# invictus717/MetaTransformer

Hardware: AMD Instinct MI355X
Metric: encoder samples/sec at B=256,N=197,C=768 (Base) (higher is better)
Workload: dtype bf16; 1 GPU; BASELINE config 2: Meta-Transformer-Base forward+backward+AdamW, tokens [256,197,768] bf16 per GPU, 12L/768d/12h, fp32 master weights, random init N(0,0.02); mode=train, per_gpu_batch=256, global_batch=256, parallelism=single

## Files before the change

### metatransformer_amd/csrc/api.hip

```cpp
#include "common.h"
#include <stdarg.h>
#include <mutex>
#include <vector>

static thread_local char g_err[512] = "";

void me_set_error(const char* fmt, ...) {
    va_list ap;
    va_start(ap, fmt);
    vsnprintf(g_err, sizeof(g_err), fmt, ap);
    va_end(ap);
}

extern "C" int me_abi_version(void) { return ME_ABI_VERSION; }
extern "C" const char* me_last_error(void) { return g_err; }
extern "C" const char* me_build_arch(void) { return "gfx950"; }

extern "C" int me_device_info(int dev, int* num_cus, int* lds_bytes, int* clock_mhz, char* name, int name_len) {
    hipDeviceProp_t prop;
    hipError_t e = hipGetDeviceProperties(&prop, dev);
    if (e != hipSuccess) {
        me_set_error("me_device_info: %s", hipGetErrorString(e));
        return ME_ERR_HIP;
    }
    if (num_cus) *num_cus = prop.multiProcessorCount;
    if (lds_bytes) *lds_bytes = (int)prop.maxSharedMemoryPerMultiProcessor;
    if (clock_mhz) *clock_mhz = prop.clockRate / 1000;
    if (name && name_len > 0) {
        snprintf(name, (size_t)name_len, "%s (%s)", prop.name, prop.gcnArchName);
    }
    return ME_OK;
}

namespace {
struct ProfEntry { int op, dt; int64_t M, N, K; hipEvent_t e0, e1; int plan; };
std::mutex g_prof_mu;
std::vector<ProfEntry> g_prof;
bool g_prof_on = false;
}

ProfScope::ProfScope(int op_, int dt_, int64_t M_, int64_t N_, int64_t K_, hipStream_t s) : stream(s), op(op_), dt(dt_), M(M_), N(N_), K(K_) {
    if (!g_prof_on) return;
    if (hipEventCreate(&e0) != hipSuccess) { e0 = nullptr; return; }
    (void)hipEventRecord(e0, stream);
}
ProfScope::~ProfScope() {
    if (!e0) return;
    hipEvent_t e1 = nullptr;
    if (hipEventCreate(&e1) != hipSuccess) { (void)hipEventDestroy(e0); return; }
    (void)hipEventRecord(e1, stream);
    std::lock_guard<std::mutex> lk(g_prof_mu);
    g_prof.push_back(ProfEntry{op, dt, M, N, K, e0, e1, plan});
}

extern "C" int me_gemm_profile_enable(int on) {
    std::lock_guard<std::mutex> lk(g_prof_mu);
    for (auto& e : g_prof) { (void)hipEventDestroy(e.e0); (void)hipEventDestroy(e.e1); }
    g_prof.clear();
    g_prof_on = on != 0;
    return ME_OK;
}

extern "C" int me_gemm_profile_read(me_gemm_profile_rec* out, int max) {
    std::lock_guard<std::mutex> lk(g_prof_mu);
    int n = 0;
    for (auto& e : g_prof) {
        float ms = 0.f;
        (void)hipEventSynchronize(e.e1);
        (void)hipEventElapsedTime(&ms, e.e0, e.e1);
        if (out && n < max) out[n] = me_gemm_profile_rec{e.op, e.dt, e.M, e.N, e.K, ms, e.plan};
        ++n;
        (void)hipEventDestroy(e.e0);
        (void)hipEventDestroy(e.e1);
    }
    g_prof.clear();
    return n;
}
```

### metatransformer_amd/csrc/block.hip

```cpp
#include "gemm_host.h"
#include "attention_host.h"
#include <string.h>
#include <stdlib.h>
#include <atomic>
#include <map>
#include <mutex>

namespace {

struct SideCtx {
    hipStream_t side = nullptr;
    hipEvent_t fork[4] = {nullptr, nullptr, nullptr, nullptr}, join = nullptr;
    bool failed = false;
};
std::atomic<int> g_wgrad_overlap{1};
bool wgrad_overlap_on() { return g_wgrad_overlap.load() != 0; }
constexpr size_t kMaxSideCtx = 64;
SideCtx* side_ctx(hipStream_t main) {
    static std::mutex mu;
    static std::map<std::pair<int, hipStream_t>, SideCtx> ctxs;
    hipStreamCaptureStatus st = hipStreamCaptureStatusNone;
    if (hipStreamIsCapturing(main, &st) != hipSuccess || st != hipStreamCaptureStatusNone) return nullptr;
    int dev = 0;
    if (hipStreamGetDevice(main, &dev) != hipSuccess) (void)hipGetDevice(&dev);
// ... 2 lines not shown
    SideCtx& c = ctxs[std::make_pair(dev, main)];
    if (c.failed) return nullptr;
    if (!c.side) {
        int cur = dev;
        (void)hipGetDevice(&cur);
        if (cur != dev && hipSetDevice(dev) != hipSuccess) { c.failed = true; return nullptr; }
        bool ok = hipStreamCreateWithFlags(&c.side, hipStreamNonBlocking) == hipSuccess;
        for (int i = 0; ok && i < 4; ++i) ok = hipEventCreateWithFlags(&c.fork[i], hipEventDisableTiming) == hipSuccess;
        ok = ok && hipEventCreateWithFlags(&c.join, hipEventDisableTiming) == hipSuccess;
        if (cur != dev) (void)hipSetDevice(cur);
        if (!ok) { c.failed = true; c.side = nullptr; return nullptr; }
    }
    return &c;
}

inline size_t align256(size_t v) { return (v + 255) & ~(size_t)255; }

struct Dims {
    int64_t M;
    int C, C3, Hd, hd;
    size_t esz, rsz;
};
int get_dims(const me_block_desc* d, Dims& s, const char* fn) {
    ME_CHECK_ARG(d != nullptr, "%s: null descriptor", fn);
    ME_CHECK_ARG((me_dtype_ok(d->dtype) || d->dtype == ME_BF16X3) && me_dtype_ok(d->res_dtype), "%s: bad dtype", fn);
    ME_CHECK_ARG(d->B > 0 && d->N > 0 && d->C > 0 && d->heads > 0 && d->hidden > 0 && d->C % d->heads == 0,
                 "%s: bad shape B=%d N=%d C=%d heads=%d hidden=%d", fn, d->B, d->N, d->C, d->heads, d->hidden);
    s.M = (int64_t)d->B * d->N;
    s.C = d->C; s.C3 = 3 * d->C; s.Hd = d->hidden; s.hd = d->C / d->heads;
    s.esz = d->dtype == ME_BF16X3 ? 6 : me_dtype_size(d->dtype); s.rsz = me_dtype_size(d->res_dtype);
// ... 43 lines not shown
        if (cs) g.colsum_a = reinterpret_cast<float*>(dummy_mem);
        const size_t b = me_gemm_workspace_bytes(&g);
        if (b > w) w = b;
    };
    probe(ME_GEMM_NT, s.M, s.C3, s.C, d->dtype, false);
    probe(ME_GEMM_NT, s.M, s.C, s.C, d->res_dtype, false);
    probe(ME_GEMM_NT, s.M, s.Hd, s.C, d->dtype, false);
    probe(ME_GEMM_NT, s.M, s.C, s.Hd, d->res_dtype, false);
    if (backward) {
        probe(ME_GEMM_NT, s.M, s.C, s.C3, d->dtype, false);
        probe(ME_GEMM_NT, s.M, s.C, s.Hd, d->dtype, false);
        probe(ME_GEMM_TN, s.C3, s.C, s.M, ME_F32, true);
        probe(ME_GEMM_TN, s.C, s.C, s.M, ME_F32, true);
        probe(ME_GEMM_TN, s.Hd, s.C, s.M, ME_F32, true);
        probe(ME_GEMM_TN, s.C, s.Hd, s.M, ME_F32, true);
    }
    return align256(w);
}

size_t aux_scratch(const Dims& s) {
    size_t a = me_layernorm_bwd_workspace(s.C), b = me_colsum_workspace(s.Hd > s.C3 ? s.Hd : s.C3);
    return align256(a > b ? a : b);
}

bool wants_fold(const me_block_desc* d) {
    return d->dtype != ME_BF16X3 && d->qkv_wf && d->fc1_wf && d->qkv_s && d->qkv_c && d->fc1_s && d->fc1_c && d->res_dtype == d->dtype;
}
size_t stats_scratch(const Dims& s) { return 2 * align256(me_row_stats_partial_bytes(s.M, s.C)) + 2 * align256((size_t)s.M * 8); }
bool emits_stats(const me_block_desc* d, const Dims& s) {
    if (!wants_fold(d) || d->gamma1 || d->gamma2 || s.C % ME_STATS_GROUP) return false;
// ... 406 lines not shown
        if (!dW && !dB) return ME_OK;
        int r = fork(fk);
        if (r) return r;
        if (dW) {
            gemm_desc(g, ME_GEMM_TN, dt, n_out, n_in, s.M, dOut, n_out, In, n_in, dW, n_in, gr->w_dtype);
            g.beta = beta; g.workspace = wgws; g.workspace_bytes = (int64_t)gsz;
            const bool fuse = dB && me_gemm_fuses_colsum(&g);
            if (fuse) g.colsum_a = dB;
            r = me_gemm(&g, wstream);
            if (r) return r;
            if (fuse) return ME_OK;
        }
        if (dB) return me_colsum(dOut, dt, n_out, s.M, n_out, dB, gr->accumulate, waws, wstream);
        return ME_OK;
    };

    const void* dyc = dy;
    if (rdt != dt) {
        if ((rc = me_cast(dy, rdt, dy_c, dt, s.M * s.C, stream))) return rc;
        dyc = dy_c;
    }
    if ((rc = wgrad(0, dyc, s.C, v.a, s.Hd, gr->fc2_w, gr->fc2_b))) return join(rc);
    if ((rc = nt(dyc, s.C, d->fc2_wt, dh, s.Hd, v.hpre))) return join(rc);
    if ((rc = wgrad(1, dh, s.Hd, v.xn2, s.C, gr->fc1_w, gr->fc1_b))) return join(rc);
    if ((rc = nt(dh, s.Hd, d->fc1_wt, dxn, s.C, nullptr))) return join(rc);
    rc = me_ln_bwd_deferred(dxn, dt, v.x1, rdt, v.mean2, v.rstd2, d->ln2_g, dy, rdt, dx1, rdt, gr->ln2_g, gr->ln2_b, gr->accumulate, s.M,
                            s.C, ln2_ws, stream, &folds[0]);
    if (rc) return join(rc);
    const void* dx1c = dx1;
    if (rdt != dt) {
        if ((rc = me_cast(dx1, rdt, dx1_c, dt, s.M * s.C, stream))) return join(rc);
        dx1c = dx1_c;
    }
    if ((rc = wgrad(2, dx1c, s.C, v.o, s.C, gr->proj_w, gr->proj_b))) return join(rc);
    if ((rc = nt(dx1c, s.C, d->proj_wt, dout, s.C, nullptr))) return join(rc);
    rc = me_attention_bwd(v.qkv, s.C3, v.o, s.C, dout, s.C, v.lse, delta, dqkv, s.C3, d->B, d->N, d->heads, s.hd, d->scale, dt, 0.f, 0, stream);
    if (rc) return join(rc);
    if ((rc = wgrad(3, dqkv, s.C3, v.xn1, s.C, gr->qkv_w, gr->qkv_b))) return join(rc);
    if ((rc = nt(dqkv, s.C3, d->qkv_wt, dxn, s.C, nullptr))) return join(rc);
    rc = me_ln_bwd_deferred(dxn, dt, x, rdt, v.mean1, v.rstd1, d->ln1_g, dx1, rdt, dx, rdt, gr->ln1_g, gr->ln1_b, gr->accumulate, s.M, s.C,
                            aws, stream, &folds[1]);
    if (rc) return join(rc);
    return join(me_ln_bwd_fold_sets(folds, 2, s.C, stream));
}

extern "C" int me_block_bwd_overlap(int enable) {
    const int prev = wgrad_overlap_on() ? 1 : 0;
    g_wgrad_overlap.store(enable ? 1 : 0);
    return prev;
}

extern "C" int me_encoder_fwd(const me_block_desc* blocks, int n_blocks, const void* x, void* y, void* pingpong, void* workspace,
                              size_t workspace_bytes, void* stream) {
// ... 37 lines not shown
```

### metatransformer_amd/csrc/common.h

```cpp
#pragma once
constexpr int ME_POL_LN_ST = 0;
constexpr int ME_POL_LN_LD = 0;
constexpr int ME_POL_ATTN_ST = 0;
constexpr int ME_POL_SLAB = 0;
#define ME_NT_LOAD(POL, ptr) ((POL) ? __builtin_nontemporal_load(ptr) : *(ptr))
#define ME_NT_STORE(POL, val, ptr) do { if (POL) __builtin_nontemporal_store((val), (ptr)); else *(ptr) = (val); } while (0)
#include <hip/hip_runtime.h>
#include <stdint.h>
#include <stdio.h>
#include "../../include/metaenc.h"

typedef __bf16 bf16_t;
typedef __attribute__((ext_vector_type(8))) __bf16 bf16x8;
typedef __attribute__((ext_vector_type(4))) __bf16 bf16x4;
typedef __attribute__((ext_vector_type(2))) __bf16 bf16x2;
typedef __attribute__((ext_vector_type(16))) float f32x16;
typedef __attribute__((ext_vector_type(4))) float f32x4;
typedef __attribute__((ext_vector_type(2))) float f32x2;
typedef __attribute__((ext_vector_type(4))) uint32_t u32x4;
constexpr float ME_GG8_LO = -0.13f, ME_GG8_STEP = 1.26f / 255.0f;
constexpr int ME_STATS_GROUP = 256;
typedef __attribute__((ext_vector_type(2))) uint32_t u32x2;

#define ME_WAVE 64
// ... 30 lines not shown
    static int n = 0;
    if (!n) {
        int dev = 0;
        (void)hipGetDevice(&dev);
        if (hipDeviceGetAttribute(&n, hipDeviceAttributeMultiprocessorCount, dev) != hipSuccess || n <= 0) n = 256;
    }
    return n;
}

struct ProfScope {
    hipEvent_t e0 = nullptr;
    hipStream_t stream;
    int op, dt;
    int64_t M, N, K;
    int plan = 0;
    ProfScope(int op, int dt, int64_t M, int64_t N, int64_t K, hipStream_t stream);
    ~ProfScope();
};

static inline size_t me_dtype_size(int dt) { return dt == ME_F32 ? 4 : dt == ME_GG8 ? 1 : 2; }
static inline bool me_dtype_ok(int dt) { return dt == ME_F32 || dt == ME_BF16; }
static inline bool me_storage_dtype_ok(int dt) { return me_dtype_ok(dt) || dt == ME_F16; }
static inline bool me_out_dtype_ok(int dt) { return me_dtype_ok(dt) || dt == ME_BF16X3; }
static inline bool me_is_planes(int dt) { return dt == ME_BF16X3 || dt == ME_BF16X2; }

constexpr int LN_FOLD_SETS = 4;
struct me_ln_fold_set { const float* partial; int nrows; float* dgamma; float* dbeta; int accumulate; };
struct me_ln_fold_batch { me_ln_fold_set set[LN_FOLD_SETS]; int cols; };
int me_ln_bwd_deferred(const void* dy, int dy_dtype, const void* x, int x_dtype, const float* mean, const float* rstd, const float* gamma,
                       const void* dres, int dres_dtype, void* dx, int dx_dtype, float* dgamma, float* dbeta, int accumulate_affine,
// ... 179 lines not shown
```

### metatransformer_amd/csrc/gemm.hip

```cpp
#include "gemm_common.h"
#include <string.h>
#include <algorithm>
#include <atomic>

namespace {

constexpr int BM = 128;
constexpr int BN = 128;
constexpr int ROWB = 128;
constexpr int TILE_BYTES = BM * ROWB;
constexpr int NT = 256;

__device__ __forceinline__ int lds_off(int row, int byteoff) {
    const int chunk = byteoff >> 4;
    return row * ROWB + (((chunk ^ ((row >> 1) & 7)) << 4) | (byteoff & 15));
}

struct Stage { u32x4 v[4]; };

template <typename T>
__device__ __forceinline__ void load_nt(Stage& s, const T* __restrict__ S, int64_t ld, int64_t nrows, int64_t K,
                                        int64_t r0, int64_t k0, int tid) {
    constexpr int E = 16 / sizeof(T);
#pragma unroll
// ... 333 lines not shown
                if (!gelu && res == 2) ME_FOLD(true, 2, 1, false, false);
            }
        }
        if (p.beta == 0.0f && !colsum_out && !bias && !gelu && res == 0) {
            if (p.c_dtype == ME_BF16) ME_FOLD(false, 0, 0, false, false);
            else ME_FOLD(false, 0, 1, false, false);
        }
    }
#undef ME_FOLD
    if (p.act == ME_ACT_NONE && !p.preact && !p.aux && !p.row_affine)
        hipLaunchKernelGGL(splitk_reduce_kernel<true>, grid, dim3(256), 0, stream, p, slabs, S, cs_part, n_part, colsum_out, sstride);
    else
        hipLaunchKernelGGL(splitk_reduce_kernel<false>, grid, dim3(256), 0, stream, p, slabs, S, cs_part, n_part, colsum_out, sstride);
}

struct GemmPlan {
    GemmFamily family = GEMM_G128;
    int bn = 0;
    int bm = 128;
    int kstep = 0;
    int split_k = 1;
    int ksteps_per_split = 0;
    size_t ws_bytes = 0;
    int64_t tail_rows = 0;
    int tail_split = 1, tail_ksteps = 0;
    int sk_wgs = 0, sk_upt = 0, sk_levels = 0, sk_l1 = 0;
};

std::atomic<int> g_reserved_cus{0};

// ... 33 lines not shown
        const int64_t tiles = ((d->M + 255) / 256) * ((d->N + 255) / 256);
        const int nkt = (int)((d->K + 63) / 64);
        const int reserved = g_reserved_cus.load();
        const int slots = 256 - (reserved > 0 ? (reserved < 128 ? reserved : 128) : 0);
        int s = (int)(slots / tiles);
        if (s < 1) s = 1;
        int ktp = (nkt + s - 1) / s;
        ktp += ktp & 1;
        if (ktp < 2) ktp = 2;
        pl.ksteps_per_split = ktp;
        pl.split_k = (nkt + ktp - 1) / ktp;
        int slabs = pl.split_k;
        const int upt = (nkt + 1) / 2;
        const int S = (int)(slots / tiles), E = (int)(slots - S * tiles);
        if (reserved > 0 && S >= 1 && E > 0 && tiles * upt >= 2 * (int64_t)slots && tiles * upt < (1ll << 30)) {
            int L1 = (int)(tiles * upt / slots);
            {
                auto tail = [&](int l1) { return S * l1 > upt ? (int64_t)1 << 40 : std::max<int64_t>(l1, (tiles * (int64_t)(upt - S * l1) + E - 1) / E); };
                if (tail(L1 + 1) < tail(L1)) L1 += 1;
            }
            const int Ul = upt - S * L1;
            int smax = S;
            for (int t = 0; t < (int)tiles; ++t) smax = std::max(smax, S + sk_left_parts(t, E, Ul, tiles * (int64_t)Ul));
            if (allow_sk && L1 >= 1) { pl.sk_wgs = slots; pl.sk_upt = upt; pl.sk_levels = S; pl.sk_l1 = L1; pl.split_k = smax; }
            slabs = std::max(slabs, smax);
        }
        pl.ws_bytes = (size_t)slabs * (size_t)g3_tn_slab_stride(d->M, d->N) * sizeof(float);
        if (d->colsum_a)
            pl.ws_bytes += (size_t)slabs * (size_t)((d->N + 255) / 256) * (size_t)d->M * sizeof(float);
    } else if (d->op == ME_GEMM_TN) {
        pl.bn = (d->N % 256 == 0 || d->N > 512) ? 256 : 128;
        const int64_t tiles = pl.bn == 256 ? t256 : t128;
        int s = (int)(SLOTS / tiles);
        if (s < 1) s = 1;
        const int min_steps = 512 / pl.kstep;
// ... 284 lines not shown
}

int gemm_fill_params(const me_gemm_desc* d, GemmParams& p) { return fill_params(d, p); }

extern "C" int me_gemm(const me_gemm_desc* d, void* stream_) {
    hipStream_t stream = reinterpret_cast<hipStream_t>(stream_);
    ProfScope prof(d ? d->op : 0, d ? d->ab_dtype : 0, d ? d->M : 0, d ? d->N : 0, d ? d->K : 0, stream);
    return gemm_impl(d, stream, &prof.plan);
}

int gemm_tn_with_launcher(const me_gemm_desc* d, hipStream_t stream, GemmTnLaunch launch, const void* ctx) {
    ProfScope prof(d ? d->op : 0, d ? d->ab_dtype : 0, d ? d->M : 0, d ? d->N : 0, d ? d->K : 0, stream);
    return gemm_impl(d, stream, &prof.plan, launch, ctx);
}

extern "C" int me_gemm_reserve_cus(int cus) {
    const int c = cus < 0 ? 0 : (cus > 128 ? 128 : cus);
    return g_reserved_cus.exchange(c);
}

extern "C" size_t me_gemm_workspace_bytes(const me_gemm_desc* d) {
    GemmRoute r;
    return route_gemm(d, r) == ME_OK ? r.pl.ws_bytes : 0;
}

int gemm_tn_is_g3(const me_gemm_desc* d) {
    GemmRoute r;
    return d && d->op == ME_GEMM_TN && route_gemm(d, r) == ME_OK && r.pl.family == GEMM_G3;
}

// ... 28 lines not shown
```

### metatransformer_amd/csrc/gemm3.hip

```cpp
#include "gemm3_core.h"

namespace {
constexpr int G3_ROWOP_AHEAD = 4;
constexpr int G3_ROWOP_AHEAD_HALF = 4;
constexpr int G3_ROWOP_AHEAD_STATS = 4;

template <int EPI, bool WRAP = false>
__global__ __launch_bounds__(512) __attribute__((amdgpu_waves_per_eu(2, 2))) void gemm_g3_kernel(const GemmParams p) {
    extern __shared__ __attribute__((aligned(16))) char smem[];
    const int tid = threadIdx.x, lane = tid & 63;
    const int wave = __builtin_amdgcn_readfirstlane(tid >> 6);
    const int wr = wave >> 2;

    const int nwg = gridDim.x, bid = blockIdx.x;
    const int xcd = bid & 7, slot = bid >> 3;
    const int F = p.g3_full_tiles;
    const int nf = (F >> 3) + (xcd < (F & 7) ? 1 : 0);
    const int base_f = xcd * (F >> 3) + (xcd < (F & 7) ? xcd : (F & 7));
    int tile, part = -1;
    if (slot < nf) {
        tile = base_f + slot;
    } else {
        const int base_all = xcd * (nwg >> 3) + (xcd < (nwg & 7) ? xcd : (nwg & 7));
        const int tid_ = base_all - base_f + (slot - nf);
// ... 698 lines not shown
            c0 += __shfl_xor(c0, 16, 64); c0 += __shfl_xor(c0, 32, 64);
            c1 += __shfl_xor(c1, 16, 64); c1 += __shfl_xor(c1, 32, 64);
            if (lane < 16) {
                float* row = p.colsum_ws + (int64_t)cs_row * p.M;
                const int wcol = wave & 3;
                const int64_t ma = m0 + wr * 128 + wcol * 16 + lane, mb = ma + 64;
                if (ma < p.M) row[ma] = c0;
                if (mb < p.M) row[mb] = c1;
            }
        }
        g3_epilogue<5>(p, s, m0, n0, g3_lane_now(), reinterpret_cast<float*>(p.C) + (int64_t)part * p.slab_stride, 0);
        u0 = ue;
    }
}


unsigned* g3r_tickets(hipStream_t stream) {
    constexpr int SETS = 64, SET_WORDS = 8 * 16;
    struct Pool {
        unsigned* base = nullptr;
        bool failed = false;
        int next = 0;
        std::map<hipStream_t, int> idx;
    };
    static std::mutex mu;
    static std::map<int, Pool> pools;
    hipStreamCaptureStatus st = hipStreamCaptureStatusNone;
    if (hipStreamIsCapturing(stream, &st) != hipSuccess || st != hipStreamCaptureStatusNone) return nullptr;
    int dev = 0;
    if (hipStreamGetDevice(stream, &dev) != hipSuccess) (void)hipGetDevice(&dev);
// ... 76 lines not shown
    const int nwg = p.tiles_m * p.tiles_n * p.split_k;
    hipLaunchKernelGGL(gemm_g3tn_kernel, dim3((unsigned)nwg), dim3(512), G3_LDS, stream, p);
    ME_CHECK_LAUNCH("me_gemm(g3 tn)");
    return ME_OK;
}

int launch_g3_tn_sk(const GemmParams& p, hipStream_t stream) {
    static OncePerDevice once;
    if (once.need())
        (void)hipFuncSetAttribute(reinterpret_cast<const void*>(&gemm_g3tn_sk_kernel), hipFuncAttributeMaxDynamicSharedMemorySize, G3_LDS);
    hipLaunchKernelGGL(gemm_g3tn_sk_kernel, dim3((unsigned)p.sk_wgs), dim3(512), G3_LDS, stream, p);
    ME_CHECK_LAUNCH("me_gemm(g3 tn, balanced partition)");
    return ME_OK;
}

bool g3_tn_supported(const GemmParams& p) {
    return p.M % 8 == 0 && p.N % 8 == 0 && p.lda % 8 == 0 && p.ldb % 8 == 0 && p.K * p.lda * 2 < (1ll << 31) &&
           p.K * p.ldb * 2 < (1ll << 31);
}

bool g3_supported(const GemmParams& p, int op) {
    if (op != ME_GEMM_NT) return false;
    if (p.K % (2 * G3_BK) != 0 || p.N % 8 != 0) return false;
    if (256 * p.lda * 2 >= (1ll << 31) || 256 * p.ldb * 2 >= (1ll << 31)) return false;
    return true;
}

int g3_cu_count() { return device_cus(); }

G3Form g3_form(const GemmParams& p, int cus) {
// ... 61 lines not shown
```

### metatransformer_amd/csrc/gemm_common.h

```cpp
#pragma once
#include "common.h"
#include "gemm_host.h"

struct GemmParams {
    const void* A; const void* B; void* C;
    int64_t M, N, K, lda, ldb, ldc;
    int c_dtype, act;
    int flags;
    float alpha, beta;
    const float* bias; const float* colscale;
    void* preact; int64_t ldpre; int preact_dtype;
    const void* aux; int64_t ldaux; int aux_dtype;
    const void* residual; int64_t ldres; int res_dtype;
    int64_t res_row_mod, out_group_rows, out_group_stride, out_row_offset;
    int tiles_m, tiles_n;
    int split_k, ksteps_per_split;
    float* colsum_ws;
    int g3_full_tiles, g3_split, g3_ktp;
    float* g3_slabs;
    int g3_half;
    unsigned* g3_tickets;
    int64_t slab_stride;
    const float* row_affine;
    int row_nparts; float row_eps;
    const float* col_shift;
    int sk_wgs, sk_upt, sk_levels, sk_l1;
    int a_wrap_kt;
    float* row_stats;
};


__host__ __device__ static inline int sk_owner(int64_t u, int E, int64_t TUl) { return (int)(((u + 1) * E - 1) / TUl); }
__host__ __device__ static inline int sk_first(int tile, int E, int Ul, int64_t TUl) { return sk_owner((int64_t)tile * Ul, E, TUl); }
__host__ __device__ static inline int sk_left_parts(int tile, int E, int Ul, int64_t TUl) {
    return Ul > 0 ? sk_owner((int64_t)(tile + 1) * Ul - 1, E, TUl) - sk_first(tile, E, Ul, TUl) + 1 : 0;
}
#define ME_SK_PARTS(p, tile) ((p).sk_levels + sk_left_parts((tile), (p).sk_wgs - (p).sk_levels * (p).tiles_m * (p).tiles_n, (p).sk_upt - (p).sk_levels * (p).sk_l1, \
                                                            (int64_t)(p).tiles_m * (p).tiles_n * ((p).sk_upt - (p).sk_levels * (p).sk_l1)))

__device__ __forceinline__ void epilogue_quad(const GemmParams& p, int64_t m, int64_t n, f32x4 v) {
    v *= p.alpha;
    if (p.row_affine) v = v * p.row_affine[2 * m] + *reinterpret_cast<const f32x4*>(p.col_shift + n) * p.row_affine[2 * m + 1];
    if (p.bias) v += *reinterpret_cast<const f32x4*>(p.bias + n);
    if (p.flags & ME_GEMM_SAVE_GELU_GRAD) {
        f32x4 dv;
        gelu_erf_pair4(v, v, dv);
        store4_from_f32(p.preact, p.preact_dtype, m * p.ldpre + n, dv);
    } else {
        if (p.preact) store4_from_f32(p.preact, p.preact_dtype, m * p.ldpre + n, v);
        if (p.act == ME_ACT_GELU) v = gelu_for4(v, p.c_dtype);
    }
// ... 186 lines not shown
};
struct G3Form {
    G3Kernel kernel = G3_UNSUPPORTED;
    int epi = 4;
    int repi = -1, pre = G3_PRE_NONE;
    int G = 0;
    int nwg = 0;
};
G3Form g3_form(const GemmParams& p, int cus);
int g3_cu_count();
int launch_g3(const GemmParams& p, const G3Form& f, hipStream_t stream);
int launch_g3_tn(const GemmParams& p, hipStream_t stream);
int launch_g3_tn_sk(const GemmParams& p, hipStream_t stream);
bool g3_tn_supported(const GemmParams& p);
static inline int64_t g3_tn_slab_stride(int64_t M, int64_t N) { return M * N; }
```

### metatransformer_amd/csrc/gemm_host.h

```cpp
#pragma once
#include "common.h"

struct GemmParams;

int gemm_fill_params(const me_gemm_desc* d, GemmParams& p);
typedef int (*GemmTnLaunch)(const GemmParams& p, hipStream_t stream, const void* ctx);
int gemm_tn_with_launcher(const me_gemm_desc* d, hipStream_t stream, GemmTnLaunch launch, const void* ctx);
int gemm_tn_is_g3(const me_gemm_desc* d);
int gemm_tn_x3_planes(const me_gemm_desc* d, hipStream_t stream);
```

Before: 8545 samples/s.

## Group paired weight-gradient GEMMs into one stream-K split launch

```diff
diff --git a/metatransformer_amd/csrc/api.hip b/metatransformer_amd/csrc/api.hip
--- a/metatransformer_amd/csrc/api.hip
+++ b/metatransformer_amd/csrc/api.hip
@@ -33,7 +33,7 @@
 }
 
 namespace {
-struct ProfEntry { int op, dt; int64_t M, N, K; hipEvent_t e0, e1; int plan; };
+struct ProfEntry { int op, dt; int64_t M, N, K; hipEvent_t e0, e1; int plan; float share = 1.0f; bool owns = true; };
 std::mutex g_prof_mu;
 std::vector<ProfEntry> g_prof;
 bool g_prof_on = false;
@@ -50,12 +50,19 @@
     if (hipEventCreate(&e1) != hipSuccess) { (void)hipEventDestroy(e0); return; }
     (void)hipEventRecord(e1, stream);
     std::lock_guard<std::mutex> lk(g_prof_mu);
+    if (M2 > 0) {
+        const double w1 = (double)M * (double)N * (double)K, w2 = (double)M2 * (double)N2 * (double)K2;
+        const float f1 = (float)(w1 / (w1 + w2));
+        g_prof.push_back(ProfEntry{op, dt, M, N, K, e0, e1, plan, f1, false});
+        g_prof.push_back(ProfEntry{op, dt, M2, N2, K2, e0, e1, plan, 1.0f - f1, true});
+        return;
+    }
     g_prof.push_back(ProfEntry{op, dt, M, N, K, e0, e1, plan});
 }
 
 extern "C" int me_gemm_profile_enable(int on) {
     std::lock_guard<std::mutex> lk(g_prof_mu);
-    for (auto& e : g_prof) { (void)hipEventDestroy(e.e0); (void)hipEventDestroy(e.e1); }
+    for (auto& e : g_prof) if (e.owns) { (void)hipEventDestroy(e.e0); (void)hipEventDestroy(e.e1); }
     g_prof.clear();
     g_prof_on = on != 0;
     return ME_OK;
@@ -68,8 +75,9 @@
         float ms = 0.f;
         (void)hipEventSynchronize(e.e1);
         (void)hipEventElapsedTime(&ms, e.e0, e.e1);
-        if (out && n < max) out[n] = me_gemm_profile_rec{e.op, e.dt, e.M, e.N, e.K, ms, e.plan};
+        if (out && n < max) out[n] = me_gemm_profile_rec{e.op, e.dt, e.M, e.N, e.K, ms * e.share, e.plan};
         ++n;
+        if (!e.owns) continue;
         (void)hipEventDestroy(e.e0);
         (void)hipEventDestroy(e.e1);
     }
diff --git a/metatransformer_amd/csrc/block.hip b/metatransformer_amd/csrc/block.hip
--- a/metatransformer_amd/csrc/block.hip
+++ b/metatransformer_amd/csrc/block.hip
@@ -2,6 +2,7 @@
 #include "attention_host.h"
 #include <string.h>
 #include <stdlib.h>
+#include <algorithm>
 #include <atomic>
 #include <map>
 #include <mutex>
@@ -40,6 +41,21 @@
     return &c;
 }
 
+constexpr int kGroupAttn = 1, kGroupMlp = 2;
+constexpr int kWgradGroupDefault = kGroupAttn;
+int wgrad_group_mask() {
+    static const int mask = [] {
+        const char* e = getenv("ME_WGRAD_GROUP");
+        if (!e) return kWgradGroupDefault;
+        if (!strcmp(e, "0")) return 0;
+        if (!strcmp(e, "attn")) return kGroupAttn;
+        if (!strcmp(e, "mlp")) return kGroupMlp;
+        if (!strcmp(e, "all")) return kGroupAttn | kGroupMlp;
+        return kWgradGroupDefault;
+    }();
+    return mask;
+}
+
 inline size_t align256(size_t v) { return (v + 255) & ~(size_t)255; }
 
 struct Dims {
@@ -113,6 +129,16 @@
         probe(ME_GEMM_TN, s.C, s.C, s.M, ME_F32, true);
         probe(ME_GEMM_TN, s.Hd, s.C, s.M, ME_F32, true);
         probe(ME_GEMM_TN, s.C, s.Hd, s.M, ME_F32, true);
+        if (d->dtype == ME_BF16 && wgrad_group_mask()) {
+            static char dummy_mem[64] __attribute__((aligned(64)));
+            me_gemm_desc h;
+            auto tn = [&](me_gemm_desc& q, int64_t M, int64_t N) {
+                gemm_desc(q, ME_GEMM_TN, ME_BF16, M, N, s.M, dummy_mem, M, dummy_mem, N, dummy_mem, N, ME_F32);
+                q.colsum_a = reinterpret_cast<float*>(dummy_mem);
+            };
+            if (wgrad_group_mask() & kGroupMlp) { tn(g, s.C, s.Hd); tn(h, s.Hd, s.C); w = std::max(w, gemm_tn_group_workspace_bytes(&g, &h)); }
+            if (wgrad_group_mask() & kGroupAttn) { tn(g, s.C, s.C); tn(h, s.C3, s.C); w = std::max(w, gemm_tn_group_workspace_bytes(&g, &h)); }
+        }
     }
     return align256(w);
 }
@@ -549,15 +575,42 @@
         if (dB) return me_colsum(dOut, dt, n_out, s.M, n_out, dB, gr->accumulate, waws, wstream);
         return ME_OK;
     };
+    struct WPair { const void* dOut; int64_t n_out; const void* In; int64_t n_in; void* dW; float* dB; };
+    auto pair_desc = [&](me_gemm_desc& q, const WPair& w) {
+        gemm_desc(q, ME_GEMM_TN, dt, w.n_out, w.n_in, s.M, w.dOut, w.n_out, w.In, w.n_in, w.dW, w.n_in, gr->w_dtype);
+        q.beta = beta; q.colsum_a = w.dB;
+    };
+    auto groupable = [&](int which, const WPair& a, const WPair& b) -> bool {
+        if (!(wgrad_group_mask() & which) || dt != ME_BF16 || !a.dW || !b.dW) return false;
+        me_gemm_desc qa, qb;
+        pair_desc(qa, a); pair_desc(qb, b);
+        const size_t need = gemm_tn_group_workspace_bytes(&qa, &qb);
+        return need > 0 && need <= gsz;
+    };
+    auto wgrad2 = [&](int fk, const WPair& a, const WPair& b) -> int {
+        int r = fork(fk);
+        if (r) return r;
+        me_gemm_desc qa, qb;
+        pair_desc(qa, a); pair_desc(qb, b);
+        r = gemm_tn_group(&qa, &qb, wgws, gsz, reinterpret_cast<hipStream_t>(wstream));
+        if (r != ME_ERR_UNSUPPORTED) return r;
+        if ((r = wgrad(fk, a.dOut, a.n_out, a.In, a.n_in, a.dW, a.dB))) return r;
+        return wgrad(fk, b.dOut, b.n_out, b.In, b.n_in, b.dW, b.dB);
+    };
 
     const void* dyc = dy;
     if (rdt != dt) {
         if ((rc = me_cast(dy, rdt, dy_c, dt, s.M * s.C, stream))) return rc;
         dyc = dy_c;
     }
-    if ((rc = wgrad(0, dyc, s.C, v.a, s.Hd, gr->fc2_w, gr->fc2_b))) return join(rc);
+    const WPair w_fc2 = {dyc, s.C, v.a, s.Hd, gr->fc2_w, gr->fc2_b}, w_fc1 = {dh, s.Hd, v.xn2, s.C, gr->fc1_w, gr->fc1_b};
+    const WPair w_proj = {rdt != dt ? dx1_c : dx1, s.C, v.o, s.C, gr->proj_w, gr->proj_b}, w_qkv = {dqkv, s.C3, v.xn1, s.C, gr->qkv_w, gr->qkv_b};
+    const int gmask = wgrad_group_mask();
+    const bool all_ok = (!(gmask & kGroupMlp) || groupable(kGroupMlp, w_fc2, w_fc1)) && (!(gmask & kGroupAttn) || groupable(kGroupAttn, w_proj, w_qkv));
+    const bool group_mlp = all_ok && (gmask & kGroupMlp), group_attn = all_ok && (gmask & kGroupAttn);
+    if (!group_mlp && (rc = wgrad(0, dyc, s.C, v.a, s.Hd, gr->fc2_w, gr->fc2_b))) return join(rc);
     if ((rc = nt(dyc, s.C, d->fc2_wt, dh, s.Hd, v.hpre))) return join(rc);
-    if ((rc = wgrad(1, dh, s.Hd, v.xn2, s.C, gr->fc1_w, gr->fc1_b))) return join(rc);
+    if ((rc = group_mlp ? wgrad2(1, w_fc2, w_fc1) : wgrad(1, dh, s.Hd, v.xn2, s.C, gr->fc1_w, gr->fc1_b))) return join(rc);
     if ((rc = nt(dh, s.Hd, d->fc1_wt, dxn, s.C, nullptr))) return join(rc);
     rc = me_ln_bwd_deferred(dxn, dt, v.x1, rdt, v.mean2, v.rstd2, d->ln2_g, dy, rdt, dx1, rdt, gr->ln2_g, gr->ln2_b, gr->accumulate, s.M,
                             s.C, ln2_ws, stream, &folds[0]);
@@ -567,11 +620,11 @@
         if ((rc = me_cast(dx1, rdt, dx1_c, dt, s.M * s.C, stream))) return join(rc);
         dx1c = dx1_c;
     }
-    if ((rc = wgrad(2, dx1c, s.C, v.o, s.C, gr->proj_w, gr->proj_b))) return join(rc);
+    if (!group_attn && (rc = wgrad(2, dx1c, s.C, v.o, s.C, gr->proj_w, gr->proj_b))) return join(rc);
     if ((rc = nt(dx1c, s.C, d->proj_wt, dout, s.C, nullptr))) return join(rc);
     rc = me_attention_bwd(v.qkv, s.C3, v.o, s.C, dout, s.C, v.lse, delta, dqkv, s.C3, d->B, d->N, d->heads, s.hd, d->scale, dt, 0.f, 0, stream);
     if (rc) return join(rc);
-    if ((rc = wgrad(3, dqkv, s.C3, v.xn1, s.C, gr->qkv_w, gr->qkv_b))) return join(rc);
+    if ((rc = group_attn ? wgrad2(3, w_proj, w_qkv) : wgrad(3, dqkv, s.C3, v.xn1, s.C, gr->qkv_w, gr->qkv_b))) return join(rc);
     if ((rc = nt(dqkv, s.C3, d->qkv_wt, dxn, s.C, nullptr))) return join(rc);
     rc = me_ln_bwd_deferred(dxn, dt, x, rdt, v.mean1, v.rstd1, d->ln1_g, dx1, rdt, dx, rdt, gr->ln1_g, gr->ln1_b, gr->accumulate, s.M, s.C,
                             aws, stream, &folds[1]);
diff --git a/metatransformer_amd/csrc/common.h b/metatransformer_amd/csrc/common.h
--- a/metatransformer_amd/csrc/common.h
+++ b/metatransformer_amd/csrc/common.h
@@ -68,6 +68,7 @@
     int op, dt;
     int64_t M, N, K;
     int plan = 0;
+    int64_t M2 = 0, N2 = 0, K2 = 0;
     ProfScope(int op, int dt, int64_t M, int64_t N, int64_t K, hipStream_t stream);
     ~ProfScope();
 };
diff --git a/metatransformer_amd/csrc/gemm.hip b/metatransformer_amd/csrc/gemm.hip
--- a/metatransformer_amd/csrc/gemm.hip
+++ b/metatransformer_amd/csrc/gemm.hip
@@ -371,6 +371,57 @@
         hipLaunchKernelGGL(splitk_reduce_kernel<false>, grid, dim3(256), 0, stream, p, slabs, S, cs_part, n_part, colsum_out, sstride);
 }
 
+__device__ __forceinline__ void fold_colsum_group(const G3TnGroupParams& g, const G3TnMember& mb, int tile_base) {
+    __shared__ float red[8][32];
+    const int nblk = (int)((mb.M + 31) / 32);
+    const int nwg = (int)(gridDim.x * gridDim.y);
+    const int b = nwg - 1 - (int)(blockIdx.y * gridDim.x + blockIdx.x);
+    if (b < nblk || nwg < nblk) {
+        const int n_part = mb.parts * mb.tiles_n;
+        for (int cb = b; cb < nblk; cb += nwg) {
+            const int64_t m = (int64_t)cb * 32 + (threadIdx.x & 31);
+            const int jg = threadIdx.x >> 5;
+            float s = 0.f;
+            if (m < mb.M) {
+                const int t0 = tile_base + (int)(m >> 8) * mb.tiles_n;
+                for (int j = jg; j < n_part; j += 8) {
+                    const bool ok = j / mb.tiles_n < wgrad_group_parts(t0 + j % mb.tiles_n, g.T, g.levels, g.left_wgs, g.left_upt);
+                    if (ok) s += mb.colsum_ws[(int64_t)j * mb.M + m];
+                }
+            }
+            red[jg][threadIdx.x & 31] = s;
+            __syncthreads();
+            if (threadIdx.x < 32 && m < mb.M) {
+                float t = 0.f;
+#pragma unroll
+                for (int k = 0; k < 8; ++k) t += red[k][threadIdx.x];
+                mb.colsum_out[m] = mb.beta != 0.0f ? t + mb.beta * mb.colsum_out[m] : t;
+            }
+            __syncthreads();
+        }
+    }
+}
+template <int CST>
+__global__ __launch_bounds__(256) void splitk_fold_group_kernel(const G3TnGroupParams g) {
+    const bool second = blockIdx.z != 0;
+    const G3TnMember& mb = second ? g.m[1] : g.m[0];
+    const int tile_base = second ? g.t0 : 0;
+    if (mb.colsum_out) fold_colsum_group(g, mb, tile_base);
+    const int q = (int)blockIdx.x * 64 + (int)(threadIdx.x & 63);
+    if (q >= (int)(mb.N / 4)) return;
+    const int64_t n = (int64_t)q * 4;
+    for (int64_t m = (int64_t)blockIdx.y * 4 + (threadIdx.x >> 6); m < mb.M; m += (int64_t)gridDim.y * 4) {
+        f32x4 c4 = {0.f, 0.f, 0.f, 0.f};
+        if (CST == 2) c4 = *reinterpret_cast<const f32x4*>(reinterpret_cast<const float*>(mb.C) + m * mb.ldc + n);
+        if (CST == 0 && mb.beta != 0.0f) c4 = load4_as_f32(mb.C, mb.c_dtype, m * mb.ldc + n);
+        const int St = wgrad_group_parts(tile_base + (int)(m >> 8) * mb.tiles_n + (int)blockIdx.x, g.T, g.levels, g.left_wgs, g.left_upt);
+        f32x4 v = fold_slabs(mb.slabs + m * mb.N + n, St, mb.slab_stride);
+        if (CST != 1) v += mb.beta * c4;
+        if (CST == 0) store4_from_f32(mb.C, mb.c_dtype, m * mb.ldc + n, v);
+        else *reinterpret_cast<f32x4*>(reinterpret_cast<float*>(mb.C) + m * mb.ldc + n) = v;
+    }
+}
+
 struct GemmPlan {
     GemmFamily family = GEMM_G128;
     int bn = 0;
@@ -434,11 +485,7 @@
         const int upt = (nkt + 1) / 2;
         const int S = (int)(slots / tiles), E = (int)(slots - S * tiles);
         if (reserved > 0 && S >= 1 && E > 0 && tiles * upt >= 2 * (int64_t)slots && tiles * upt < (1ll << 30)) {
-            int L1 = (int)(tiles * upt / slots);
-            {
-                auto tail = [&](int l1) { return S * l1 > upt ? (int64_t)1 << 40 : std::max<int64_t>(l1, (tiles * (int64_t)(upt - S * l1) + E - 1) / E); };
-                if (tail(L1 + 1) < tail(L1)) L1 += 1;
-            }
+            const int L1 = sk_balanced_l1(tiles, upt, slots, S, E, nullptr);
             const int Ul = upt - S * L1;
             int smax = S;
             for (int t = 0; t < (int)tiles; ++t) smax = std::max(smax, S + sk_left_parts(t, E, Ul, tiles * (int64_t)Ul));
@@ -753,6 +800,70 @@
     return gemm_impl(d, stream, &prof.plan, launch, ctx);
 }
 
+namespace {
+bool tn_group_plan(const me_gemm_desc* d0, const me_gemm_desc* d1, GemmRoute (&r)[2], WgradGroupPlan& gp) {
+    if (!d0 || !d1) return false;
+    const me_gemm_desc* d[2] = {d0, d1};
+    for (int j = 0; j < 2; ++j) {
+        const me_gemm_desc* q = d[j];
+        if (q->op != ME_GEMM_TN || q->ab_dtype != ME_BF16 || q->alpha != 1.0f || !me_dtype_ok(q->c_dtype) || q->bias || q->colscale || q->preact ||
+            q->aux || q->residual || q->act != ME_ACT_NONE || q->flags || q->res_row_mod || q->out_group_rows || q->row_affine || q->row_parts ||
+            q->row_stats || q->col_shift || q->a_wrap_k)
+            return false;
+        if (route_gemm(q, r[j]) != ME_OK || r[j].pl.family != GEMM_G3) return false;
+    }
+    if (d0->K != d1->K || d0->c_dtype != d1->c_dtype || (d0->beta != 0.0f) != (d1->beta != 0.0f)) return false;
+    gp = plan_wgrad_group(d0->M, d0->N, d1->M, d1->N, d0->K, 256);
+    return gp.ok;
+}
+}
+
+size_t gemm_tn_group_workspace_bytes(const me_gemm_desc* d0, const me_gemm_desc* d1) {
+    GemmRoute r[2];
+    WgradGroupPlan gp;
+    return tn_group_plan(d0, d1, r, gp) ? gp.ws_bytes : 0;
+}
+
+int gemm_tn_group(const me_gemm_desc* d0, const me_gemm_desc* d1, void* workspace, size_t workspace_bytes, hipStream_t stream) {
+    GemmRoute r[2];
+    WgradGroupPlan gp;
+    if (g_reserved_cus.load() != 0 || !tn_group_plan(d0, d1, r, gp) || !workspace || workspace_bytes < gp.ws_bytes || (uintptr_t)workspace % 16 != 0) return ME_ERR_UNSUPPORTED;
+    const me_gemm_desc* d[2] = {d0, d1};
+    ProfScope prof(ME_GEMM_TN, ME_BF16, d0->M, d0->N, d0->K, stream);
+    prof.M2 = d1->M; prof.N2 = d1->N; prof.K2 = d1->K;
+    prof.plan = (GEMM_G3 & 15) | 16 | (gp.left_wgs ? 32 : 0) | 64 | (std::max(gp.parts[0], gp.parts[1]) << 8);
+    G3TnGroupParams g;
+    memset(&g, 0, sizeof(g));
+    float* const ws = reinterpret_cast<float*>(workspace);
+    for (int j = 0; j < 2; ++j) {
+        G3TnMember& m = g.m[j];
+        m.A = d[j]->A; m.B = d[j]->B;
+        m.slabs = ws + gp.slab_off[j];
+        m.colsum_ws = d[j]->colsum_a ? ws + gp.cs_off[j] : nullptr;
+        m.C = d[j]->C; m.colsum_out = d[j]->colsum_a;
+        m.M = d[j]->M; m.N = d[j]->N; m.K = d[j]->K; m.lda = d[j]->lda; m.ldb = d[j]->ldb; m.ldc = d[j]->ldc;
+        m.slab_stride = d[j]->M * d[j]->N;
+        m.tiles_m = (int)((d[j]->M + 255) / 256); m.tiles_n = (int)((d[j]->N + 255) / 256);
+        m.c_dtype = d[j]->c_dtype; m.parts = gp.parts[j]; m.beta = d[j]->beta;
+    }
+    g.t0 = gp.tiles[0]; g.T = gp.T;
+    g.levels = gp.levels; g.l1 = gp.l1; g.left_wgs = gp.left_wgs; g.left_upt = gp.left_upt;
+    const int rc = launch_g3_tn_group(g, gp.wgs, stream);
+    if (rc) return rc;
+    const int64_t Nmax = std::max(d0->N, d1->N), Mmax = std::max(d0->M, d1->M);
+    const unsigned gx = (unsigned)((Nmax / 4 + 63) / 64);
+    int64_t gy = (Mmax + 3) / 4;
+    const int64_t cap = 4096 / gx > 1 ? 4096 / gx : 1;
+    if (gy > cap) gy = cap;
+    const dim3 grid(gx, (unsigned)gy, 2);
+    const bool f32 = d0->c_dtype == ME_F32, acc = d0->beta != 0.0f || d1->beta != 0.0f;
+    if (!f32) hipLaunchKernelGGL(splitk_fold_group_kernel<0>, grid, dim3(256), 0, stream, g);
+    else if (acc) hipLaunchKernelGGL(splitk_fold_group_kernel<2>, grid, dim3(256), 0, stream, g);
+    else hipLaunchKernelGGL(splitk_fold_group_kernel<1>, grid, dim3(256), 0, stream, g);
+    ME_CHECK_LAUNCH("me_gemm(g3 tn grouped fold)");
+    return ME_OK;
+}
+
 extern "C" int me_gemm_reserve_cus(int cus) {
     const int c = cus < 0 ? 0 : (cus > 128 ? 128 : cus);
     return g_reserved_cus.exchange(c);
diff --git a/metatransformer_amd/csrc/gemm3.hip b/metatransformer_amd/csrc/gemm3.hip
--- a/metatransformer_amd/csrc/gemm3.hip
+++ b/metatransformer_amd/csrc/gemm3.hip
@@ -736,6 +736,95 @@
     }
 }
 
+__device__ __forceinline__ GemmParams g3tn_member_params(const G3TnGroupParams& g, bool second) {
+    GemmParams p = {};
+    p.A = second ? g.m[1].A : g.m[0].A;
+    p.B = second ? g.m[1].B : g.m[0].B;
+    p.C = second ? g.m[1].slabs : g.m[0].slabs;
+    p.colsum_ws = second ? g.m[1].colsum_ws : g.m[0].colsum_ws;
+    p.M = second ? g.m[1].M : g.m[0].M;
+    p.N = second ? g.m[1].N : g.m[0].N;
+    p.K = second ? g.m[1].K : g.m[0].K;
+    p.lda = second ? g.m[1].lda : g.m[0].lda;
+    p.ldb = second ? g.m[1].ldb : g.m[0].ldb;
+    p.slab_stride = second ? g.m[1].slab_stride : g.m[0].slab_stride;
+    p.tiles_m = second ? g.m[1].tiles_m : g.m[0].tiles_m;
+    p.tiles_n = second ? g.m[1].tiles_n : g.m[0].tiles_n;
+    p.alpha = 1.0f;
+    return p;
+}
+__global__ __launch_bounds__(512) __attribute__((amdgpu_waves_per_eu(2, 2))) void gemm_g3tn_group_kernel(const G3TnGroupParams g) {
+    extern __shared__ __attribute__((aligned(16))) char smem[];
+    const int tid = threadIdx.x, lane = tid & 63;
+    const int wave = __builtin_amdgcn_readfirstlane(tid >> 6);
+    const int wr = wave >> 2;
+    const int nwg = gridDim.x, bid = blockIdx.x;
+    const int xcd = bid & 7, q = nwg >> 3, r = nwg & 7;
+    const int wgid = (xcd < r ? xcd * (q + 1) : r * (q + 1) + (xcd - r) * q) + (bid >> 3);
+    int64_t u0, u1;
+    wgrad_group_units(wgid, g.T, g.levels, g.left_wgs, g.left_upt, &u0, &u1);
+    u0 = __builtin_amdgcn_readfirstlane((int)u0);
+    u1 = __builtin_amdgcn_readfirstlane((int)u1);
+    G3State s;
+    while (u0 < u1) {
+        const WgradGroupSeg seg = wgrad_group_seg(wgid, u0, u1, g.T, g.levels, g.l1, g.left_wgs, g.left_upt);
+        const int gtile = __builtin_amdgcn_readfirstlane(seg.gtile), kt0 = __builtin_amdgcn_readfirstlane(seg.kt0);
+        const int kt1 = __builtin_amdgcn_readfirstlane(seg.kt1), part = __builtin_amdgcn_readfirstlane(seg.part);
+        const int64_t ue = __builtin_amdgcn_readfirstlane((int)seg.ue);
+        const bool second = gtile >= g.t0;
+        const int tile = second ? gtile - g.t0 : gtile;
+        const GemmParams p = g3tn_member_params(g, second);
+        const int tm = __builtin_amdgcn_readfirstlane(tile / p.tiles_n), tn = tile - tm * p.tiles_n;
+        const int cs_row = part * p.tiles_n + tn;
+        const int64_t m0 = (int64_t)tm * G3_BM, n0 = (int64_t)tn * G3_BN;
+        g3_init_lane_tn(s, p, smem, wave, g3_lane_now());
+        const G3Src null = g3_null_src(p);
+        const G3Src src = g3_make_src_tn(p, tm, tn);
+        g3_zero(s);
+        g3_issue<0>(s, src, 0, kt0); g3_issue<1>(s, src, 0, kt0); g3_issue<2>(s, src, 0, kt0); g3_issue<3>(s, src, 0, kt0);
+        g3_issue<0>(s, src, 1, kt0 + 1); g3_issue<1>(s, src, 1, kt0 + 1); g3_issue<2>(s, src, 1, kt0 + 1);
+        asm volatile("s_waitcnt vmcnt(6)" ::: "memory");
+        __builtin_amdgcn_s_barrier();
+        if (wr == 1) __builtin_amdgcn_s_barrier();
+        const bool do_cs = p.colsum_ws != nullptr;
+        s.cs[0] = s.cs[1] = 0.f;
+        int cs_turn = (tn + p.tiles_n - ((kt0 >> 1) % p.tiles_n)) % p.tiles_n;
+        auto my_turn = [&]() {
+            if (!do_cs) return false;
+            const bool mine = cs_turn == 0;
+            cs_turn = mine ? p.tiles_n - 1 : cs_turn - 1;
+            return mine;
+        };
+        for (int kt = kt0; kt < kt1 - 2; kt += 2) {
+            const bool c = my_turn();
+            g3_ktile<0, true>(s, src, kt + 1, src, kt + 2, c);
+            g3_ktile<1, true>(s, src, kt + 2, src, kt + 3, c);
+        }
+        {
+            const bool c = my_turn();
+            g3_ktile<0, true>(s, src, kt1 - 1, null, 0, c);
+            g3_ktile<1, true>(s, null, 0, null, 0, c);
+        }
+        asm volatile("s_waitcnt vmcnt(0)" ::: "memory");
+        if (wr == 0) __builtin_amdgcn_s_barrier();
+        if (do_cs) {
+            float c0 = s.cs[0], c1 = s.cs[1];
+            c0 += __shfl_xor(c0, 16, 64); c0 += __shfl_xor(c0, 32, 64);
+            c1 += __shfl_xor(c1, 16, 64); c1 += __shfl_xor(c1, 32, 64);
+            if (g3_lane_now() < 16) {
+                float* row = p.colsum_ws + (int64_t)cs_row * p.M;
+                const int wcol = wave & 3;
+                const int64_t ma = m0 + wr * 128 + wcol * 16 + g3_lane_now(), mb = ma + 64;
+                if (ma < p.M) row[ma] = c0;
+                if (mb < p.M) row[mb] = c1;
+            }
+        }
+        g3_epilogue<5>(p, s, m0, n0, g3_lane_now(), reinterpret_cast<float*>(p.C) + (int64_t)part * p.slab_stride, 0);
+        u0 = ue;
+    }
+    (void)lane;
+}
+
 
 unsigned* g3r_tickets(hipStream_t stream) {
     constexpr int SETS = 64, SET_WORDS = 8 * 16;
@@ -842,6 +931,15 @@
     return ME_OK;
 }
 
+int launch_g3_tn_group(const G3TnGroupParams& g, int wgs, hipStream_t stream) {
+    static OncePerDevice once;
+    if (once.need())
+        (void)hipFuncSetAttribute(reinterpret_cast<const void*>(&gemm_g3tn_group_kernel), hipFuncAttributeMaxDynamicSharedMemorySize, G3_LDS);
+    hipLaunchKernelGGL(gemm_g3tn_group_kernel, dim3((unsigned)wgs), dim3(512), G3_LDS, stream, g);
+    ME_CHECK_LAUNCH("me_gemm(g3 tn, grouped)");
+    return ME_OK;
+}
+
 bool g3_tn_supported(const GemmParams& p) {
     return p.M % 8 == 0 && p.N % 8 == 0 && p.lda % 8 == 0 && p.ldb % 8 == 0 && p.K * p.lda * 2 < (1ll << 31) &&
            p.K * p.ldb * 2 < (1ll << 31);
diff --git a/metatransformer_amd/csrc/gemm_common.h b/metatransformer_amd/csrc/gemm_common.h
--- a/metatransformer_amd/csrc/gemm_common.h
+++ b/metatransformer_amd/csrc/gemm_common.h
@@ -1,6 +1,7 @@
 #pragma once
 #include "common.h"
 #include "gemm_host.h"
+#include "wgrad_plan.h"
 
 struct GemmParams {
     const void* A; const void* B; void* C;
@@ -30,11 +31,6 @@
 };
 
 
-__host__ __device__ static inline int sk_owner(int64_t u, int E, int64_t TUl) { return (int)(((u + 1) * E - 1) / TUl); }
-__host__ __device__ static inline int sk_first(int tile, int E, int Ul, int64_t TUl) { return sk_owner((int64_t)tile * Ul, E, TUl); }
-__host__ __device__ static inline int sk_left_parts(int tile, int E, int Ul, int64_t TUl) {
-    return Ul > 0 ? sk_owner((int64_t)(tile + 1) * Ul - 1, E, TUl) - sk_first(tile, E, Ul, TUl) + 1 : 0;
-}
 #define ME_SK_PARTS(p, tile) ((p).sk_levels + sk_left_parts((tile), (p).sk_wgs - (p).sk_levels * (p).tiles_m * (p).tiles_n, (p).sk_upt - (p).sk_levels * (p).sk_l1, \
                                                             (int64_t)(p).tiles_m * (p).tiles_n * ((p).sk_upt - (p).sk_levels * (p).sk_l1)))
 
@@ -251,3 +247,19 @@
 int launch_g3_tn_sk(const GemmParams& p, hipStream_t stream);
 bool g3_tn_supported(const GemmParams& p);
 static inline int64_t g3_tn_slab_stride(int64_t M, int64_t N) { return M * N; }
+
+struct G3TnMember {
+    const void* A; const void* B;
+    float* slabs; float* colsum_ws;
+    void* C; float* colsum_out;
+    int64_t M, N, K, lda, ldb, ldc, slab_stride;
+    int tiles_m, tiles_n, c_dtype;
+    int parts;
+    float beta;
+};
+struct G3TnGroupParams {
+    G3TnMember m[2];
+    int t0, T;
+    int levels, l1, left_wgs, left_upt;
+};
+int launch_g3_tn_group(const G3TnGroupParams& g, int wgs, hipStream_t stream);
diff --git a/metatransformer_amd/csrc/gemm_host.h b/metatransformer_amd/csrc/gemm_host.h
--- a/metatransformer_amd/csrc/gemm_host.h
+++ b/metatransformer_amd/csrc/gemm_host.h
@@ -7,4 +7,6 @@
 typedef int (*GemmTnLaunch)(const GemmParams& p, hipStream_t stream, const void* ctx);
 int gemm_tn_with_launcher(const me_gemm_desc* d, hipStream_t stream, GemmTnLaunch launch, const void* ctx);
 int gemm_tn_is_g3(const me_gemm_desc* d);
+size_t gemm_tn_group_workspace_bytes(const me_gemm_desc* d0, const me_gemm_desc* d1);
+int gemm_tn_group(const me_gemm_desc* d0, const me_gemm_desc* d1, void* workspace, size_t workspace_bytes, hipStream_t stream);
 int gemm_tn_x3_planes(const me_gemm_desc* d, hipStream_t stream);
diff --git a/metatransformer_amd/csrc/wgrad_plan.h b/metatransformer_amd/csrc/wgrad_plan.h
--- /dev/null
+++ b/metatransformer_amd/csrc/wgrad_plan.h
@@ -0,0 +1,116 @@
+#pragma once
+#include <stdint.h>
+#include <stddef.h>
+
+#if defined(__HIPCC__) || defined(__CUDACC__)
+#define ME_HD __host__ __device__
+#else
+#define ME_HD
+#endif
+
+ME_HD static inline int sk_owner(int64_t u, int E, int64_t TUl) { return (int)(((u + 1) * E - 1) / TUl); }
+ME_HD static inline int sk_first(int tile, int E, int Ul, int64_t TUl) { return sk_owner((int64_t)tile * Ul, E, TUl); }
+ME_HD static inline int sk_left_parts(int tile, int E, int Ul, int64_t TUl) {
+    return Ul > 0 ? sk_owner((int64_t)(tile + 1) * Ul - 1, E, TUl) - sk_first(tile, E, Ul, TUl) + 1 : 0;
+}
+static inline int sk_balanced_l1(int64_t tiles, int upt, int slots, int S, int E, int64_t* tail_out) {
+    auto tail = [&](int l1) -> int64_t {
+        if ((int64_t)S * l1 > upt) return (int64_t)1 << 40;
+        const int64_t left = (tiles * (int64_t)(upt - S * l1) + E - 1) / E;
+        return left > l1 ? left : l1;
+    };
+    int L1 = (int)(tiles * upt / slots);
+    if (tail(L1 + 1) < tail(L1)) L1 += 1;
+    if (tail_out) *tail_out = tail(L1);
+    return L1;
+}
+
+struct WgradGroupPlan {
+    bool ok = false;
+    int tiles[2] = {0, 0};
+    int T = 0, upt = 0;
+    int wgs = 0, levels = 0, l1 = 0, left_wgs = 0, left_upt = 0;
+    int parts[2] = {0, 0};
+    size_t slab_off[2] = {0, 0};
+    size_t cs_off[2] = {0, 0};
+    size_t ws_bytes = 0;
+};
+ME_HD static inline int wgrad_group_parts(int tile, int T, int levels, int left_wgs, int left_upt) {
+    return levels + (left_wgs > 0 ? sk_left_parts(tile, left_wgs, left_upt, (int64_t)T * left_upt) : 0);
+}
+struct WgradGroupSeg { int gtile, kt0, kt1, part; int64_t ue; };
+ME_HD static inline void wgrad_group_units(int wgid, int T, int levels, int left_wgs, int left_upt, int64_t* u0, int64_t* u1) {
+    *u0 = 0; *u1 = 1;
+    if (wgid < levels * T) return;
+    const int e = wgid - levels * T;
+    const int64_t TUl = (int64_t)T * left_upt;
+    if (e >= left_wgs) { *u1 = 0; return; }
+    *u0 = (int64_t)e * TUl / left_wgs;
+    *u1 = (int64_t)(e + 1) * TUl / left_wgs;
+}
+ME_HD static inline WgradGroupSeg wgrad_group_seg(int wgid, int64_t u0, int64_t u1, int T, int levels, int l1, int left_wgs, int left_upt) {
+    WgradGroupSeg s;
+    if (wgid < levels * T) {
+        const int level = wgid / T;
+        s.gtile = wgid - level * T;
+        s.kt0 = level * l1 * 2; s.kt1 = s.kt0 + l1 * 2;
+        s.part = level;
+        s.ue = u1;
+    } else {
+        s.gtile = (int)(u0 / left_upt);
+        const int64_t tu0 = (int64_t)s.gtile * left_upt;
+        s.ue = u1 < tu0 + left_upt ? u1 : tu0 + left_upt;
+        s.kt0 = (levels * l1 + (int)(u0 - tu0)) * 2; s.kt1 = (levels * l1 + (int)(s.ue - tu0)) * 2;
+        s.part = levels + (wgid - levels * T) - sk_first(s.gtile, left_wgs, left_upt, (int64_t)T * left_upt);
+    }
+    return s;
+}
+static inline WgradGroupPlan plan_wgrad_group(int64_t M0, int64_t N0, int64_t M1, int64_t N1, int64_t K, int slots) {
+    WgradGroupPlan g;
+    const int64_t M[2] = {M0, M1}, N[2] = {N0, N1};
+    int tn[2];
+    for (int j = 0; j < 2; ++j) {
+        if (M[j] <= 0 || N[j] <= 0) return g;
+        tn[j] = (int)((N[j] + 255) / 256);
+        const int64_t t = ((M[j] + 255) / 256) * tn[j];
+        if (t > slots) return g;
+        g.tiles[j] = (int)t;
+    }
+    g.T = g.tiles[0] + g.tiles[1];
+    const int64_t nkt = (K + 63) / 64;
+    if (K <= 0 || nkt > (1 << 24) || g.T > slots) return g;
+    g.upt = (int)((nkt + 1) / 2);
+    if ((int64_t)g.T * g.upt >= ((int64_t)1 << 30)) return g;
+    const int S0 = slots / g.T;
+    const int S = S0 < g.upt ? S0 : g.upt;
+    const int Lu = (g.upt + S - 1) / S;
+    g.levels = (g.upt + Lu - 1) / Lu;
+    g.l1 = Lu;
+    g.wgs = g.levels * g.T;
+    const int E = slots - S0 * g.T;
+    if (S == S0 && E > 0 && (int64_t)g.T * g.upt >= 2 * (int64_t)slots) {
+        int64_t tail = 0;
+        const int L1 = sk_balanced_l1(g.T, g.upt, slots, S, E, &tail);
+        const int Ul = g.upt - S * L1;
+        if (L1 >= 1 && Ul > 0 && tail * 20 <= (int64_t)Lu * 19) {
+            g.levels = S; g.l1 = L1; g.left_wgs = E; g.left_upt = Ul;
+            g.wgs = slots;
+        }
+    }
+    int t0 = 0;
+    for (int j = 0; j < 2; ++j) {
+        int pmax = g.levels;
+        for (int t = t0; t < t0 + g.tiles[j]; ++t) {
+            const int q = wgrad_group_parts(t, g.T, g.levels, g.left_wgs, g.left_upt);
+            pmax = q > pmax ? q : pmax;
+        }
+        g.parts[j] = pmax;
+        t0 += g.tiles[j];
+    }
+    size_t off = 0;
+    for (int j = 0; j < 2; ++j) { g.slab_off[j] = off; off += (size_t)g.parts[j] * (size_t)(M[j] * N[j]); }
+    for (int j = 0; j < 2; ++j) { g.cs_off[j] = off; off += (size_t)g.parts[j] * (size_t)tn[j] * (size_t)M[j]; }
+    g.ws_bytes = off * sizeof(float);
+    g.ok = true;
+    return g;
+}
```

Result: no change. 8614 samples/s, median of 6 (+0.8%).
